# lucidrains/glom-pytorch

Hardware: NVIDIA H100
Metric: column-iterations/sec (BxNxLxiters) at dim=512 L=6 224/14 (higher is better)
Workload: dtype bf16

## Files before the change

### glom_pytorch_b200/csrc/tc_common.cuh

```cuda
#pragma once
#include "engine.h"
#include "ptx.cuh"

#include <stdio.h>

namespace glom {

constexpr int BM = 128;
constexpr int BK = 64;
constexpr uint32_t A_STAGE_BYTES = BM * BK * 2;

constexpr int STG_PITCH = 68;
constexpr uint32_t STG_BYTES = 32 * STG_PITCH * 4;
template <int S, int R>
__device__ __forceinline__ void stage_write_step(const float (&acc)[R], float* stg, int warp_in_wg, int lane) {
  const int r = 16 * (warp_in_wg & 1) + (lane >> 2), c = 2 * (lane & 3);
#pragma unroll
  for (int j = 0; j < 8; ++j) {
#pragma unroll
    for (int h = 0; h < 2; ++h)
      *reinterpret_cast<float2*>(stg + (r + 8 * h) * STG_PITCH + 8 * j + c) =
          make_float2(acc[4 * (8 * S + j) + 2 * h], acc[4 * (8 * S + j) + 2 * h + 1]);
  }
}
template <int R>
__device__ __forceinline__ void stage_write(const float (&acc)[R], float* stg, int s, int warp_in_wg, int lane) {
  static_assert(R % 32 == 0 && R <= 128, "m64 x N fragment, N in {64, 128, 256}");
  if (s == 0) stage_write_step<0>(acc, stg, warp_in_wg, lane);
  if constexpr (R >= 64) { if (s == 1) stage_write_step<1>(acc, stg, warp_in_wg, lane); }
  if constexpr (R >= 128) {
    if (s == 2) stage_write_step<2>(acc, stg, warp_in_wg, lane);
    if (s == 3) stage_write_step<3>(acc, stg, warp_in_wg, lane);
  }
}
__device__ __forceinline__ void stage_read(const float* stg, int x, int lane, uint32_t (&v)[32]) {
  const float4* src = reinterpret_cast<const float4*>(stg + lane * STG_PITCH + 32 * x);
#pragma unroll
  for (int q = 0; q < 8; ++q) {
    const float4 f = src[q];
    v[4 * q] = __float_as_uint(f.x); v[4 * q + 1] = __float_as_uint(f.y);
    v[4 * q + 2] = __float_as_uint(f.z); v[4 * q + 3] = __float_as_uint(f.w);
  }
}

template <int N, int TB>
__device__ __forceinline__ void wgmma_kblock(float (&acc)[N / 2], uint32_t a_smem, uint32_t b_smem) {
  const uint64_t ad = wgmma_desc_sw128(a_smem, 16, 1024);
  const uint64_t bd = TB ? wgmma_desc_sw128(b_smem, 8192, 1024) : wgmma_desc_sw128(b_smem, 16, 1024);
#pragma unroll
  for (int k = 0; k < BK / 16; ++k) wgmma_bf16<N, 0, TB>(acc, ad + 2 * k, bd + (TB ? (2048 >> 4) : 2) * k);
}

__device__ __forceinline__ float row_chunk_sumsq(float a, float b, float c, float d) {
  float q = a * a;
  q = fmaf(b, b, q);
  q = fmaf(c, c, q);
  q = fmaf(d, d, q);
  q += __shfl_xor_sync(0xffffffffu, q, 1);
  q += __shfl_xor_sync(0xffffffffu, q, 2);
  q += __shfl_xor_sync(0xffffffffu, q, 4);
  return q;
}

struct K2Chunk {
  int l, L, d, n, row0;
  int prow0;
  int s_bcast;
  bool remap;
  const float* s32_in; const __nv_bfloat16* c_in; const float* pos;
  float* s32_out; __nv_bfloat16* sb_out; __nv_bfloat16* sp_out;
};
template <bool FULL, bool SETTLE = false>
__device__ __forceinline__ void k2_chunk(const uint32_t (&v)[32], const float4 b4, uint8_t* patch, const K2Chunk& k,
                                         int col, int lane, int rows_left, float (&rowsq)[8], uint32_t live = ~0u,
                                         float* rowdsq = nullptr, bool want_dsq = false) {
#pragma unroll
  for (int c = 0; c < 8; ++c)
    *reinterpret_cast<uint4*>(patch + lane * 128 + ((c ^ (lane & 7)) << 4)) =
        make_uint4(v[4 * c], v[4 * c + 1], v[4 * c + 2], v[4 * c + 3]);
  __syncwarp();
  const int c = lane & 7, rsub = lane >> 3;
  const bool top = (k.l == k.L - 1);
  const bool has_td = (k.l >= 1);
  const int ld = k.L * k.d, ldp = (k.L - 1) * k.d;
  const size_t base = ((size_t)k.row0 * k.L + k.l) * k.d + col + c * 4;
  const size_t pbase = ((size_t)k.row0 * (k.L - 1) + (k.l - 1)) * k.d + col + c * 4;
#pragma unroll
  for (int h = 0; h < 2; ++h) {
    float4 sv[4], pp[4];
    uint2 cw[4];
#pragma unroll
    for (int j = 0; j < 4; ++j) {
      const int r = (h * 4 + j) * 4 + rsub;
      sv[j] = make_float4(0.f, 0.f, 0.f, 0.f); pp[j] = sv[j]; cw[j] = make_uint2(0u, 0u);
      if ((FULL || r < rows_left) && (!SETTLE || ((live >> r) & 1u))) {
        size_t so = base + (unsigned)(r * ld);
        if (!SETTLE && k.remap) {
          int sr = k.prow0 + r;
          if (k.n >= 32) { if (sr >= k.n) sr -= k.n; } else sr %= k.n;
          so = (size_t)k.l * k.d + col + c * 4 + (unsigned)(sr * ld);
        }
        sv[j] = k.s_bcast ? __ldg(reinterpret_cast<const float4*>(k.s32_in + (size_t)k.l * k.d + col + c * 4))
                          : __ldcs(reinterpret_cast<const float4*>(k.s32_in + so));
        cw[j] = __ldcs(reinterpret_cast<const uint2*>(k.c_in + so));
        if (has_td) {
          int pr = k.prow0 + r;
          if (k.n >= 32) { if (pr >= k.n) pr -= k.n; } else pr %= k.n;
          pp[j] = __ldg(reinterpret_cast<const float4*>(k.pos + (size_t)pr * k.d + col + c * 4));
        }
      }
    }
#pragma unroll
    for (int j = 0; j < 4; ++j) {
      const int i = h * 4 + j;
      const int r = i * 4 + rsub;
      const float4 acc = *reinterpret_cast<const float4*>(patch + r * 128 + ((c ^ (r & 7)) << 4));
      float o0 = (sv[j].x + (acc.x + b4.x)) + __uint_as_float(cw[j].x << 16);
      float o1 = (sv[j].y + (acc.y + b4.y)) + __uint_as_float(cw[j].x & 0xFFFF0000u);
      float o2 = (sv[j].z + (acc.z + b4.z)) + __uint_as_float(cw[j].y << 16);
      float o3 = (sv[j].w + (acc.w + b4.w)) + __uint_as_float(cw[j].y & 0xFFFF0000u);
      if (top) { o0 = o0 / 3.0f; o1 = o1 / 3.0f; o2 = o2 / 3.0f; o3 = o3 / 3.0f; }
      else { o0 *= 0.25f; o1 *= 0.25f; o2 *= 0.25f; o3 *= 0.25f; }
      const bool store = (FULL || r < rows_left) && (!SETTLE || ((live >> r) & 1u));
      if constexpr (SETTLE) if (want_dsq) {
        const float e0 = store ? o0 - sv[j].x : 0.f, e1 = store ? o1 - sv[j].y : 0.f;
        const float e2 = store ? o2 - sv[j].z : 0.f, e3 = store ? o3 - sv[j].w : 0.f;
        rowdsq[i] += row_chunk_sumsq(e0, e1, e2, e3);
      }
      if (store) {
        const size_t o = base + (unsigned)(r * ld);
        __stcs(reinterpret_cast<float4*>(k.s32_out + o), make_float4(o0, o1, o2, o3));
        *reinterpret_cast<uint2*>(k.sb_out + o) = make_uint2(pack_bf16x2(o0, o1), pack_bf16x2(o2, o3));
        if (has_td)
          *reinterpret_cast<uint2*>(k.sp_out + pbase + (unsigned)(r * ldp)) =
              make_uint2(pack_bf16x2(o0 + pp[j].x, o1 + pp[j].y), pack_bf16x2(o2 + pp[j].z, o3 + pp[j].w));
      } else {
        o0 = o1 = o2 = o3 = 0.f;
      }
      rowsq[i] += row_chunk_sumsq(o0, o1, o2, o3);
    }
  }
  __syncwarp();
}

static inline int encode_map(Launch& ln, CUtensorMap* m, const void* base, int rank, const uint64_t* dims,
                             const uint64_t* strides_bytes , const uint32_t* box, const char* what) {
  cuuint64_t gd[3]; cuuint64_t gs[2]; cuuint32_t bx[3]; cuuint32_t es[3] = {1, 1, 1};
  for (int i = 0; i < rank; ++i) { gd[i] = dims[i]; bx[i] = box[i]; }
  for (int i = 0; i < rank - 1; ++i) gs[i] = strides_bytes[i];
  const CUresult r = ln.enc(m, CU_TENSOR_MAP_DATA_TYPE_BFLOAT16, (cuuint32_t)rank, const_cast<void*>(base), gd, gs, bx, es,
                         CU_TENSOR_MAP_INTERLEAVE_NONE, CU_TENSOR_MAP_SWIZZLE_128B, CU_TENSOR_MAP_L2_PROMOTION_L2_256B,
                         CU_TENSOR_MAP_FLOAT_OOB_FILL_NONE);
  if (r != CUDA_SUCCESS) return ln.fail(GLOM_B200_ERR_CUDA, "cuTensorMapEncodeTiled(%s) failed with CUresult %d", what, (int)r);
  return 0;
}

static inline int map2d(Launch& ln, CUtensorMap* m, const void* base, uint64_t rows, uint64_t cols, uint32_t box_rows,
                        const char* what) {
  const uint64_t dims[2] = {cols, rows};
  const uint64_t strides[1] = {cols * 2};
  const uint32_t box[2] = {(uint32_t)BK, box_rows};
  return encode_map(ln, m, base, 2, dims, strides, box, what);
}

}
```

### glom_pytorch_b200/csrc/tc_kernels.cu

```cuda
#include "gemm_sched.cuh"
#include "tc_common.cuh"

#include <stdio.h>
#include <stdlib.h>
#include <string.h>

#include <type_traits>

namespace glom {

constexpr int GEMM_CONSUMER_WARPS = 8;
constexpr int GEMM_THREADS = 128 + 32 * GEMM_CONSUMER_WARPS;
constexpr uint32_t GEMM_PRODUCER_REGS = 40;
constexpr uint32_t GEMM_CONSUMER_REGS = 232;

__device__ unsigned long long g_kernel_clk[PROF_KINDS][8];


template <int MODE, int BN>
struct GemmCfg {
  static constexpr int PARTS = (BN == 256) ? 4 : 2;
  static constexpr int PART_COLS = BN / PARTS;
  static constexpr int THREADS = GEMM_THREADS;
  static constexpr uint32_t B_STAGE_BYTES = BN * BK * 2;
  static constexpr uint32_t STAGE_BYTES = A_STAGE_BYTES + B_STAGE_BYTES;
  static_assert(MODE >= 0 && MODE <= 2, "0 = GEMM1+GELU, 1 = GEMM2+combine, 2 = tokeniser");
  static constexpr int STAGES = (BN == 256) ? 3 : (BN == 128) ? 4 : 5;
  static constexpr uint32_t OUT_BOX_BYTES = 64 * BK * 2;
  static constexpr uint32_t PATCH_BYTES = 4096;
  static constexpr size_t EPI_BYTES = (MODE == 0) ? 2 * (BN / 64) * (size_t)OUT_BOX_BYTES
                                                  : 4 * (size_t)STG_BYTES + (size_t)GEMM_CONSUMER_WARPS * PATCH_BYTES + 4 * 32 * 4;
  static constexpr size_t SMEM_BYTES = 1024  + (size_t)STAGES * STAGE_BYTES + EPI_BYTES + 256 ;
  static_assert(SMEM_BYTES <= 232448, "over the 227 KB of shared memory a block may opt in to");
};

__device__ __forceinline__ void tok_chunk(const uint32_t (&v)[32], const float4 b4, uint8_t* patch, float* dst,
                                          size_t pitch, int lane, int rows_left) {
#pragma unroll
  for (int c = 0; c < 8; ++c)
    *reinterpret_cast<uint4*>(patch + lane * 128 + ((c ^ (lane & 7)) << 4)) =
        make_uint4(v[4 * c], v[4 * c + 1], v[4 * c + 2], v[4 * c + 3]);
  __syncwarp();
  const int c = lane & 7, rsub = lane >> 3;
#pragma unroll
  for (int i = 0; i < 8; ++i) {
    const int r = i * 4 + rsub;
    const float4 a = *reinterpret_cast<const float4*>(patch + r * 128 + ((c ^ (r & 7)) << 4));
    if (r < rows_left)
      *reinterpret_cast<float4*>(dst + (size_t)r * pitch + c * 4) = make_float4(a.x + b4.x, a.y + b4.y, a.z + b4.z, a.w + b4.w);
  }
  __syncwarp();
}

template <int MODE>
__device__ __forceinline__ bool settle_skip(const GemmParams& p, const TileInfo& t) {
  if (p.block_frozen[t.m_blk]) return true;
  return MODE == 0 && t.z == 0 && p.block_fresh != nullptr && !p.block_fresh[t.m_blk];
}

template <int MODE, int BN, bool CNT, bool SETTLE = false>
__global__ void __launch_bounds__(GEMM_THREADS, 1)
gemm_kernel(const __grid_constant__ CUtensorMap map_a0,
            const __grid_constant__ CUtensorMap map_a1,
            const __grid_constant__ CUtensorMap map_a2,
            const __grid_constant__ CUtensorMap map_b,
            const __grid_constant__ CUtensorMap map_out,
            const GemmParams p) {
  using Cfg = GemmCfg<MODE, BN>;
  constexpr int STAGES = Cfg::STAGES;
  constexpr bool RED = MODE != 2 && !SETTLE;
  extern __shared__ uint8_t smem_raw[];
  uint8_t* smem = smem_raw + ((1024u - (smem_u32(smem_raw) & 1023u)) & 1023u);
  uint8_t* epi = smem + (size_t)STAGES * Cfg::STAGE_BYTES;
  float* stg_all = reinterpret_cast<float*>(epi);
  uint8_t* patches = epi + 4 * STG_BYTES;
  float* xch = reinterpret_cast<float*>(patches + (size_t)GEMM_CONSUMER_WARPS * Cfg::PATCH_BYTES);
  uint64_t* full_bar = reinterpret_cast<uint64_t*>(epi + Cfg::EPI_BYTES);
  uint64_t* empty_bar = full_bar + STAGES;

  const int warp = threadIdx.x >> 5;
  const int lane = threadIdx.x & 31;
  constexpr int W_TMA = 0;
  constexpr int W_CONSUMER0 = 4;
  const int cta_rank = (int)(blockIdx.x & 1);
  const int cluster_id = blockIdx.x >> 1;
  const int num_clusters = gridDim.x >> 1;

  if (warp == W_TMA && lane == 0) {
    tma_prefetch_desc(&map_a0);
    tma_prefetch_desc(&map_b);
    if (MODE == 0) { tma_prefetch_desc(&map_a1); tma_prefetch_desc(&map_a2); tma_prefetch_desc(&map_out); }
    for (int i = 0; i < STAGES; ++i) { mbar_init(&full_bar[i], 1); mbar_init(&empty_bar[i], 2 * GEMM_CONSUMER_WARPS); }
    fence_barrier_init();
  }
  cluster_sync_all();
  pdl_launch_dependents();
  pdl_wait();
  const bool clk_thread = blockIdx.x == 0 && warp == W_TMA && lane == 0;
  ClockSample* clk_s = reinterpret_cast<ClockSample*>(empty_bar + STAGES);
  if (clk_thread) *clk_s = clock_sample_begin();
  const bool cnt_cta = CNT && blockIdx.x == 0;
  unsigned long long* const cnt = g_kernel_clk[MODE == 0 ? PROF_GEMM1 : MODE == 1 ? PROF_GEMM2 : PROF_TOKENIZE];
  unsigned long long w0 = 0, w1 = 0;
#define GLOM_CNT_WAIT(acc, stmt) do { if (cnt_cta) { const long long t_ = clock64(); stmt; acc += (unsigned long long)(clock64() - t_); } else { stmt; } } while (0)

  if (warp < W_CONSUMER0) {
    setmaxnreg_dec<GEMM_PRODUCER_REGS>();
    if (warp == W_TMA) {
      const uint32_t elected = elect_one();
      int stage = 0; uint32_t phase = 0;
      const uint32_t smem0 = smem_u32(smem);
      const uint64_t pol_first = l2_policy_evict_first();
      const int kbg_n = 4 * p.d / BK;
      const int blk_skip = (p.m128 - 1) * kbg_n;
      for (int it = 0, tile; (tile = sched_tile<MODE>(p, cluster_id, num_clusters, it)) >= 0; ++it) {
        const TileInfo t = decode_tile<MODE, RED>(p, tile);
        if constexpr (SETTLE) { if (settle_skip<MODE>(p, t)) continue; }
        const CUtensorMap* amap;
        int a_col, b_row;
        if (MODE == 0) {
          const int l = t.z >> 1;
          if (t.z == 0) { amap = &map_a0; a_col = 0; }
          else if (t.z & 1) { amap = &map_a2; a_col = l * p.d; }
          else { amap = &map_a1; a_col = (l - 1) * p.d; }
          b_row = t.z * 4 * p.d + t.n_blk * BN;
        } else if (MODE == 1) {
          amap = &map_a0; a_col = 0;
          b_row = t.z * p.d + t.n_blk * BN;
        } else {
          amap = &map_a0; a_col = 0;
          b_row = t.n_blk * BN;
        }
        const int a_row = t.m_blk * 256 + cta_rank * BM;
        const int blk0 = (2 * t.z * p.m128 + (a_row >> 7)) * kbg_n;
        int td_skip = blk_skip;
        if constexpr (RED && MODE == 1) {
          if (p.num_m_rep > 0 && t.z + 1 >= p.remap_l) td_skip -= ((a_row >> 7) - (a_row >> 7) % p.h_period) * kbg_n;
        }
        for (int kb = 0; kb < t.num_kb; ++kb) {
          GLOM_CNT_WAIT(w0, mbar_wait(&empty_bar[stage], phase ^ 1));
          if (elected) {
            const uint32_t sa = smem0 + (uint32_t)stage * Cfg::STAGE_BYTES;
            uint64_t* bar = &full_bar[stage];
            mbar_arrive_expect_tx(bar, Cfg::STAGE_BYTES);
            if (MODE == 1) {
              const int blk = blk0 + kb + (kb >= kbg_n ? td_skip : 0);
              tma_load_2d_hint(sa, amap, bar, 0, blk * BM, pol_first);
            } else {
              tma_load_2d(sa, amap, bar, a_col + kb * BK, a_row);
            }
            const uint32_t b_half = (uint32_t)cta_rank * (BN / 2);
            tma_load_2d_multicast(sa + A_STAGE_BYTES + b_half * BK * 2, &map_b, bar, kb * BK, b_row + (int)b_half, 0x3);
          }
          __syncwarp();
          if (++stage == STAGES) { stage = 0; phase ^= 1; }
        }
      }
      if (cnt_cta && elected) atomicAdd(&cnt[4], w0);
    }
  } else {
    setmaxnreg_inc<GEMM_CONSUMER_REGS>();
    const int cw = warp - W_CONSUMER0;
    const int wg = cw >> 2, wi = cw & 3;
    const int pair = cw >> 1, x = cw & 1;
    float* stg = stg_all + pair * (STG_BYTES / 4);
    uint8_t* patch = patches + (size_t)cw * Cfg::PATCH_BYTES;
    float* xch_p = xch + pair * 32;
    const uint32_t smem0 = smem_u32(smem);
    const uint64_t pol_stream = l2_policy_evict_first();
    const bool st_issuer = (threadIdx.x & 127) == 0;
    const uint32_t out_wg = smem_u32(epi) + (uint32_t)wg * (BN / 64) * Cfg::OUT_BOX_BYTES;
    const uint32_t st_row = (uint32_t)(16 * wi + 8 * ((lane >> 3) & 1) + (lane & 7)) * 128;
    const int st_jx = lane >> 4, st_sw = lane & 7;
    const uint32_t empty_peer = mapa_shared(smem_u32(empty_bar), (uint32_t)cta_rank ^ 1u);
    auto release = [&](int slot) {
      __syncwarp();
      if (lane == 0) { mbar_arrive(&empty_bar[slot]); mbar_arrive_cluster(empty_peer + 8u * (uint32_t)slot); }
    };
    int stage = 0; uint32_t phase = 0;
    float acc[BN / 2];
    for (int it = 0, tile; (tile = sched_tile<MODE>(p, cluster_id, num_clusters, it)) >= 0; ++it) {
      const TileInfo t = decode_tile<MODE, RED>(p, tile);
      if constexpr (SETTLE) { if (settle_skip<MODE>(p, t)) continue; }
      const int row0 = t.m_blk * 256 + cta_rank * BM + pair * 32;
      const int rows_left = p.rows - row0;
      uint32_t live = ~0u;
      if constexpr (SETTLE && MODE == 1)
        live = __ballot_sync(0xffffffffu, row0 + lane < p.rows && !p.frozen[(row0 + lane) / p.n]);
      bool remap = false;
      if constexpr (RED && MODE == 1) remap = p.num_m_rep > 0 && t.z >= p.remap_l;
      if (MODE == 1 && lane < rows_left) {
        const int src_row = remap ? (row0 + lane) % p.n : row0 + lane;
        const size_t o = ((size_t)src_row * p.L + t.z) * p.d + t.n_blk * BN + x * (BN / 2);
#pragma unroll
        for (int c = 0; c < BN / 2; c += 32) {
          if (!p.s_bcast) prefetch_l2(p.s32_in + o + c);
          if ((c & 63) == 0) prefetch_l2(p.c_in + o + c);
        }
      }
#pragma unroll
      for (int i = 0; i < BN / 2; ++i) acc[i] = 0.f;
      int prev = -1;
      for (int kb = 0; kb < t.num_kb; ++kb) {
        GLOM_CNT_WAIT(w0, mbar_wait(&full_bar[stage], phase));
        const uint32_t sa = smem0 + (uint32_t)stage * Cfg::STAGE_BYTES;
        wgmma_fence_regs(acc);
        wgmma_fence();
        wgmma_kblock<BN, 0>(acc, sa + (uint32_t)wg * (A_STAGE_BYTES / 2), sa + A_STAGE_BYTES);
        wgmma_commit();
        wgmma_wait<1>();
        wgmma_fence_regs(acc);
        if (prev >= 0) release(prev);
        prev = stage;
        if (++stage == STAGES) { stage = 0; phase ^= 1; }
      }
      wgmma_wait<0>();
      wgmma_fence_regs(acc);
      release(prev);
      const long long busy_t0 = cnt_cta ? clock64() : 0;
      if constexpr (MODE == 0) {
        const int wrow0 = t.m_blk * 256 + cta_rank * BM + 64 * wg;
        if (wrow0 < p.rows) {
          const int hblk0 = (t.z * p.m128 + (t.m_blk * 2 + cta_rank)) * (4 * p.d / BK) + t.n_blk * (BN / BK);
          const float* bias = p.bias + (size_t)t.z * 4 * p.d + t.n_blk * BN + 2 * (lane & 3);
          uint32_t pk[BN / 4];
#pragma unroll
          for (int s = 0; s < BN / 64; ++s) {
#pragma unroll
            for (int j = 0; j < 8; ++j) {
              const float2 b = __ldg(reinterpret_cast<const float2*>(bias + 64 * s + 8 * j));
#pragma unroll
              for (int h = 0; h < 2; ++h)
                pk[16 * s + 2 * j + h] = gelu_pair_bf16(acc[4 * (8 * s + j) + 2 * h], acc[4 * (8 * s + j) + 2 * h + 1], b.x, b.y);
            }
          }
          if (st_issuer) bulk_wait_group_read<0>();
          named_bar_sync(1 + wg, 128);
#pragma unroll
          for (int s = 0; s < BN / 64; ++s)
#pragma unroll
            for (int q = 0; q < 4; ++q)
              stmatrix_x4(out_wg + (uint32_t)s * Cfg::OUT_BOX_BYTES + st_row + ((uint32_t)((2 * q + st_jx) ^ st_sw) << 4),
                          pk[16 * s + 4 * q], pk[16 * s + 4 * q + 1], pk[16 * s + 4 * q + 2], pk[16 * s + 4 * q + 3]);
          fence_proxy_async_smem();
          named_bar_sync(1 + wg, 128);
          if (st_issuer) {
#pragma unroll
            for (int s = 0; s < BN / 64; ++s)
              tma_store_2d_hint(&map_out, out_wg + (uint32_t)s * Cfg::OUT_BOX_BYTES, 0, (hblk0 + s) * BM + 64 * wg, pol_stream);
            bulk_commit_group();
          }
        }
      } else {
#pragma unroll 1
        for (int s = 0; s < BN / 64; ++s) {
          stage_write(acc, stg, s, wi, lane);
          named_bar_sync(1 + pair, 64);
          uint32_t v[32];
          stage_read(stg, x, lane, v);
          const int cc = 64 * s + 32 * x;
          if (MODE == 2) {
            float* trow = p.tok_out + (size_t)row0 * p.d + t.n_blk * BN + cc;
            const float4 b4 = __ldg(reinterpret_cast<const float4*>(p.bias + t.n_blk * BN + cc + (lane & 7) * 4));
            tok_chunk(v, b4, patch, trow, (size_t)p.d, lane, rows_left);
          } else {
            K2Chunk kc;
            kc.l = t.z; kc.L = p.L; kc.d = p.d; kc.n = p.n; kc.row0 = row0; kc.prow0 = row0 % p.n; kc.s_bcast = p.s_bcast;
            kc.remap = remap;
            kc.s32_in = p.s32_in; kc.c_in = p.c_in; kc.pos = p.pos;
            kc.s32_out = p.s32_out; kc.sb_out = p.sb_out; kc.sp_out = p.sp_out;
            const int col = t.n_blk * BN + cc;
            const float4 b4 = __ldg(reinterpret_cast<const float4*>(p.bias + (size_t)t.z * p.d + col + (lane & 7) * 4));
            float rowsq[8], rowdsq[8];
#pragma unroll
            for (int i = 0; i < 8; ++i) rowsq[i] = rowdsq[i] = 0.f;
            const bool want_dsq = SETTLE && p.dsq_out != nullptr;
            if (rows_left >= 32) k2_chunk<true, SETTLE>(v, b4, patch, kc, col, lane, 32, rowsq, live, rowdsq, want_dsq);
            else k2_chunk<false, SETTLE>(v, b4, patch, kc, col, lane, rows_left, rowsq, live, rowdsq, want_dsq);
            int part = cc / Cfg::PART_COLS;
            bool writer = true;
            if (Cfg::PART_COLS == 64) {
              float* dxch = reinterpret_cast<float*>(patches + (size_t)(cw | 1) * Cfg::PATCH_BYTES);
              if (x == 1 && (lane & 7) == 0) {
#pragma unroll
                for (int i = 0; i < 8; ++i) xch_p[i * 4 + (lane >> 3)] = rowsq[i];
                if (want_dsq) {
#pragma unroll
                  for (int i = 0; i < 8; ++i) dxch[i * 4 + (lane >> 3)] = rowdsq[i];
                }
              }
              named_bar_sync(1 + pair, 64);
              if (x == 0) {
#pragma unroll
                for (int i = 0; i < 8; ++i) rowsq[i] += xch_p[i * 4 + (lane >> 3)];
                if (want_dsq) {
#pragma unroll
                  for (int i = 0; i < 8; ++i) rowdsq[i] += dxch[i * 4 + (lane >> 3)];
                }
              }
              writer = x == 0;
            }
            if (writer && (lane & 7) == 0) {
              const size_t po = ((size_t)row0 * p.L + t.z) * p.nparts + t.n_blk * Cfg::PARTS + part;
              float* nsq = p.nsq_out + po;
              const int ldn = p.L * p.nparts;
#pragma unroll
              for (int i = 0; i < 8; ++i) {
                const int r = i * 4 + (lane >> 3);
                if (r < rows_left && (!SETTLE || ((live >> r) & 1u))) {
                  nsq[(unsigned)(r * ldn)] = rowsq[i];
                  if (want_dsq) p.dsq_out[po + (unsigned)(r * ldn)] = rowdsq[i];
                }
              }
            }
          }
          named_bar_sync(1 + pair, 64);
        }
      }
      if (cnt_cta) w1 += (unsigned long long)(clock64() - busy_t0);
    }
    if (cnt_cta && cw == 0 && lane == 0) { atomicAdd(&cnt[2], w0); atomicAdd(&cnt[6], w1); }
    if (MODE == 0 && st_issuer) bulk_wait_group<0>();
  }
#undef GLOM_CNT_WAIT

  cluster_sync_all();
  if (clk_thread) clock_sample_end(*clk_s, g_kernel_clk[MODE == 0 ? PROF_GEMM1 : MODE == 1 ? PROF_GEMM2 : PROF_TOKENIZE]);
}

constexpr int ATTN_CONSUMER_WARPS = 8;
constexpr int ATTN_THREADS = 128 + 32 * ATTN_CONSUMER_WARPS;
constexpr uint32_t ATTN_PRODUCER_REGS = 56;
constexpr uint32_t ATTN_CONSUMER_REGS = 224;
constexpr int ATTN_SCALE_WARPS = 3;
constexpr float ATTN_BOUND_MAX = 96.f;
constexpr int ATTN_SINGLE_PASS_MAX = 576;
constexpr int ATTN_PASS_KEYS = 512;

template <int KEYS>
struct AttnCfg {
  static_assert(KEYS == 128 || KEYS == 256, "S block = one wgmma N");
  static constexpr int MAX_KB = (KEYS == 256) ? 1 : 5;
  static constexpr uint32_t SLOT_BYTES = A_STAGE_BYTES + (uint32_t)KEYS * BK * 2;
  static_assert(SLOT_BYTES >= 4 * 8192, "a slot holds a V chunk");
};

struct AttnParams {
  int n, L, d;
  int attend_self, mask_side, mask_d2_max;
  int n_pad16, n_pad64, nkb, nchunk;
  int num_stages;
  int ntiles, num_items;
  int nparts;
  const float* nsq;
  __nv_bfloat16* c_out;
  float scale;
  int key0, nk, pass_first, pass_last;
  float* o_acc;
  float* ml_acc;
  const int* frozen;
  int l_full;
};

constexpr size_t attn_fixed_smem(int nchunk, int n_pad16) {
  return 1024  + (size_t)nchunk * A_STAGE_BYTES + (size_t)n_pad16 * (2 * 2 * 4 + 4) + 256;
}
static_assert(attn_fixed_smem(4, 256) + 3 * AttnCfg<256>::SLOT_BYTES <= 232448, "n = 256: three 48 KB slots");
static_assert(attn_fixed_smem(9, 576) + 2 * AttnCfg<128>::SLOT_BYTES <= 232448, "n = 576: two 32 KB slots");

__device__ __forceinline__ float attn_row_norm(const float* ns, int nparts) {
  float ss = 0.f;
  if ((nparts & 3) == 0 && nparts <= 16) {
    float4 q[4];
#pragma unroll
    for (int i = 0; i < 4; ++i)
      q[i] = 4 * i < nparts ? __ldg(reinterpret_cast<const float4*>(ns) + i) : make_float4(0.f, 0.f, 0.f, 0.f);
#pragma unroll
    for (int i = 0; i < 4; ++i) ss = (((ss + q[i].x) + q[i].y) + q[i].z) + q[i].w;
  } else {
    for (int i = 0; i < nparts; ++i) ss += ns[i];
  }
  return sqrtf(ss);
}

template <int KEYS, bool CNT, bool SETTLE = false>
__global__ void __launch_bounds__(ATTN_THREADS, 1)
attn_kernel(const __grid_constant__ CUtensorMap map_q,
            const __grid_constant__ CUtensorMap map_k,
            const __grid_constant__ CUtensorMap map_v,
            const AttnParams p) {
  using Cfg = AttnCfg<KEYS>;
  constexpr uint32_t SLOT = Cfg::SLOT_BYTES;
  extern __shared__ uint8_t smem_raw[];
  uint8_t* smem = smem_raw + ((1024u - (smem_u32(smem_raw) & 1023u)) & 1023u);
  uint8_t* p_smem = smem;
  uint8_t* stages = p_smem + (size_t)p.nchunk * A_STAGE_BYTES;
  float* sc = reinterpret_cast<float*>(stages + (size_t)p.num_stages * SLOT);
  uint32_t* key_hw = reinterpret_cast<uint32_t*>(sc + 4 * p.n_pad16);
  uint64_t* full_bar = reinterpret_cast<uint64_t*>(key_hw + p.n_pad16);
  uint64_t* empty_bar = full_bar + p.num_stages;
  uint64_t* sc_full = empty_bar + p.num_stages;
  uint64_t* sc_empty = sc_full + 2;
  ClockSample* clk_s = reinterpret_cast<ClockSample*>(sc_empty + 2);

  const int warp = threadIdx.x >> 5;
  const int lane = threadIdx.x & 31;
  constexpr int W_TMA = 0;
  constexpr int W_CONSUMER0 = 4;
  const int nsub = (p.d + 255) / 256;
  const int per_img = p.ntiles * (SETTLE ? p.L : p.l_full);
  const int full_items = p.num_items - p.ntiles * (p.L - p.l_full);
  auto item_bl = [&](int it, int& b, int& l) {
    if (SETTLE) { b = it / per_img; l = (it % per_img) / p.ntiles; }
    else attn_item(it, full_items, per_img, p.ntiles, p.l_full, b, l);
  };
  const int nkb = (KEYS == 256) ? 1 : p.nkb;
  constexpr float LOG2E = 1.4426950408889634f;

  if (warp == W_TMA && lane == 0) {
    tma_prefetch_desc(&map_q); tma_prefetch_desc(&map_k); tma_prefetch_desc(&map_v);
    for (int i = 0; i < p.num_stages; ++i) { mbar_init(&full_bar[i], 1); mbar_init(&empty_bar[i], ATTN_CONSUMER_WARPS); }
    for (int i = 0; i < 2; ++i) { mbar_init(&sc_full[i], ATTN_SCALE_WARPS); mbar_init(&sc_empty[i], ATTN_CONSUMER_WARPS); }
    fence_barrier_init();
  }
  __syncthreads();
  pdl_launch_dependents();
  pdl_wait();
  const bool clk_thread = blockIdx.x == 0 && warp == W_TMA && lane == 0;
  if (clk_thread) *clk_s = clock_sample_begin();
  const bool cnt_cta = CNT && blockIdx.x == 0;
  unsigned long long* const cnt = g_kernel_clk[PROF_ATTN];
  unsigned long long w0 = 0, w1 = 0, w2 = 0;
#define GLOM_CNT_WAIT(acc, stmt) do { if (cnt_cta) { const long long t_ = clock64(); stmt; acc += (unsigned long long)(clock64() - t_); } else { stmt; } } while (0)

  if (warp < W_CONSUMER0) {
    setmaxnreg_dec<ATTN_PRODUCER_REGS>();
    if (warp == W_TMA) {
      const uint32_t elected = elect_one();
      int stage = 0; uint32_t phase = 0;
      const uint32_t stages0 = smem_u32(stages);
      for (int it = blockIdx.x; it < p.num_items; it += gridDim.x) {
        int b, l;
        item_bl(it, b, l);
        if constexpr (SETTLE) { if (p.frozen[b]) continue; }
        const int q0 = (it % p.ntiles) * BM;
        for (int kb = 0; kb < nkb; ++kb) {
          for (int dc = 0; dc < p.d / BK; ++dc) {
// ... 230 lines not shown
              uint32_t* ptr = p_word(rbase + 8 * h, kb * KEYS + col);
              const uint32_t wv = *ptr;
              *ptr = pack_bf16x2(__uint_as_float(wv << 16) * f, __uint_as_float(wv & 0xFFFF0000u) * f);
            }
          }
        }
      }
      float l_pass[2];
#pragma unroll
      for (int h = 0; h < 2; ++h) {
        l_pass[h] = l_run[h] + __shfl_xor_sync(0xffffffffu, l_run[h], 1);
        l_pass[h] += __shfl_xor_sync(0xffffffffu, l_pass[h], 2);
      }
      fence_proxy_async_smem();
      named_bar_sync(2 + wg, 128);
      const long long cnt_t1 = cnt_cta ? clock64() : 0;
      const unsigned long long cnt_w1 = w0;
      if (cnt_cta) w1 += (unsigned long long)(cnt_t1 - cnt_t0) - (cnt_w1 - cnt_w0);

      size_t acc_row[2];
      float inv_l[2], f_old[2] = {0.f, 0.f}, f_new[2] = {1.f, 1.f};
#pragma unroll
      for (int h = 0; h < 2; ++h) {
        acc_row[h] = (img_row0 + (size_t)qi[h]) * p.L + l;
        inv_l[h] = 1.0f / l_pass[h];
        if (multi) {
          float m_acc = NEG_INF, l_acc = 0.f;
          if (!p.pass_first && qi[h] < p.n) {
            const float2 ml = *reinterpret_cast<const float2*>(p.ml_acc + acc_row[h] * 2);
            m_acc = ml.x; l_acc = ml.y;
          }
          float m_pass = exact_max ? m_run[h] : row_bound[h];
          if (l_pass[h] == 0.f) m_pass = NEG_INF;
          const float m_new = fmaxf(m_acc, m_pass);
          f_old[h] = (m_acc == NEG_INF) ? 0.f : ex2_approx(m_acc - m_new);
          f_new[h] = (m_pass == NEG_INF) ? 0.f : ex2_approx(m_pass - m_new);
          const float l_new = l_acc * f_old[h] + l_pass[h] * f_new[h];
          inv_l[h] = p.pass_last ? 1.0f / l_new : 1.0f;
          __syncwarp();
          if (!p.pass_last && (lane & 3) == 0 && qi[h] < p.n)
            *reinterpret_cast<float2*>(p.ml_acc + acc_row[h] * 2) = make_float2(m_new, l_new);
        }
      }

#pragma unroll 1
      for (int sp = 0; sp < nsub; ++sp) {
        float o[128];
#pragma unroll
        for (int i = 0; i < 128; ++i) o[i] = 0.f;
        int prev = -1;
        for (int kc = 0; kc < p.nchunk; ++kc) {
          GLOM_CNT_WAIT(w0, mbar_wait(&full_bar[stage], phase));
          const uint32_t sa = stages0 + (uint32_t)stage * SLOT;
          wgmma_fence_regs(o);
          wgmma_fence();
          wgmma_kblock<256, 1>(o, p0 + (uint32_t)kc * A_STAGE_BYTES + (uint32_t)wg * (A_STAGE_BYTES / 2), sa);
          wgmma_commit();
          wgmma_wait<1>();
          wgmma_fence_regs(o);
          if (prev >= 0) { __syncwarp(); if (lane == 0) mbar_arrive(&empty_bar[prev]); }
          prev = stage;
          if (++stage == p.num_stages) { stage = 0; phase ^= 1; }
        }
        wgmma_wait<0>();
        wgmma_fence_regs(o);
        __syncwarp();
        if (lane == 0) mbar_arrive(&empty_bar[prev]);
        if (multi) {
#pragma unroll
          for (int i = 0; i < 128; i += 2) {
            const int h = (i >> 1) & 1;
            const int col = sp * 256 + 8 * (i >> 2) + cq;
            if (col >= p.d || qi[h] >= p.n) continue;
            float v0 = o[i], v1 = o[i + 1];
            float2* accp = reinterpret_cast<float2*>(p.o_acc + acc_row[h] * p.d + col);
            float2 prev = make_float2(0.f, 0.f);
            if (!p.pass_first) prev = *accp;
            v0 = v0 * f_new[h] + prev.x * f_old[h];
            v1 = v1 * f_new[h] + prev.y * f_old[h];
            if (!p.pass_last) { *accp = make_float2(v0, v1); continue; }
            *reinterpret_cast<uint32_t*>(p.c_out + acc_row[h] * p.d + col) = pack_bf16x2(v0 * inv_l[h], v1 * inv_l[h]);
          }
        } else {
          const int q = lane & 3;
          const bool b1 = q & 1, b2 = q & 2;
#pragma unroll
          for (int h = 0; h < 2; ++h) {
            __nv_bfloat16* crow = p.c_out + acc_row[h] * p.d + sp * 256 + 8 * q;
            const bool row_ok = qi[h] < p.n;
#pragma unroll
            for (int g = 0; g < 8; ++g) {
              uint32_t a[4];
#pragma unroll
              for (int t = 0; t < 4; ++t)
                a[t] = pack_bf16x2(o[4 * (4 * g + t) + 2 * h] * inv_l[h], o[4 * (4 * g + t) + 2 * h + 1] * inv_l[h]);
#pragma unroll
              for (int pr = 0; pr < 2; ++pr) {
                const uint32_t r = __shfl_xor_sync(0xffffffffu, b1 ? a[2 * pr] : a[2 * pr + 1], 1);
                if (b1) a[2 * pr] = r; else a[2 * pr + 1] = r;
              }
#pragma unroll
              for (int pr = 0; pr < 2; ++pr) {
                const uint32_t r = __shfl_xor_sync(0xffffffffu, b2 ? a[pr] : a[2 + pr], 2);
                if (b2) a[pr] = r; else a[2 + pr] = r;
              }
              if (row_ok && sp * 256 + 32 * g < p.d)
                *reinterpret_cast<uint4*>(crow + 32 * g) = make_uint4(a[0], a[1], a[2], a[3]);
            }
          }
        }
      }
      if (cnt_cta) w2 += (unsigned long long)(clock64() - cnt_t1) - (w0 - cnt_w1);
      ++k;
    }
    if (cnt_cta && cw == 0 && lane == 0) { atomicAdd(&cnt[5], w0); atomicAdd(&cnt[6], w1); atomicAdd(&cnt[7], w2); }
  }
#undef GLOM_CNT_WAIT

  __syncthreads();
  if (clk_thread) clock_sample_end(*clk_s, g_kernel_clk[PROF_ATTN]);
}

cudaError_t tc_kernel_clocks(unsigned long long* out , bool reset) {
  cudaError_t e = cudaMemcpyFromSymbol(out, g_kernel_clk, sizeof(unsigned long long) * PROF_KINDS * 8);
  if (e == cudaSuccess && reset) {
    static const unsigned long long zeros[PROF_KINDS * 8] = {};
    e = cudaMemcpyToSymbol(g_kernel_clk, zeros, sizeof(zeros));
  }
  return e;
}

template <int MODE, int BN, bool CNT, bool SETTLE = false>
static cudaError_t launch_gemm_impl(const CUtensorMap& a0, const CUtensorMap& a1, const CUtensorMap& a2, const CUtensorMap& bm,
                                    const CUtensorMap& out, const GemmParams& p, int num_sms, cudaStream_t st);

static bool count_waits() {
  static const bool on = [] { const char* ev = getenv("GLOM_B200_WAIT_COUNTERS"); return ev && ev[0] == '1'; }();
  return on;
}

template <int MODE, int BN>
static cudaError_t launch_gemm(const CUtensorMap& a0, const CUtensorMap& a1, const CUtensorMap& a2, const CUtensorMap& bm,
                               const CUtensorMap& out, const GemmParams& p, int num_sms, cudaStream_t st) {
  if constexpr (MODE != 2) {
    if (p.block_frozen) return launch_gemm_impl<MODE, BN, false, true>(a0, a1, a2, bm, out, p, num_sms, st);
  }
  if (count_waits()) return launch_gemm_impl<MODE, BN, true>(a0, a1, a2, bm, out, p, num_sms, st);
  return launch_gemm_impl<MODE, BN, false>(a0, a1, a2, bm, out, p, num_sms, st);
}

template <int MODE, int BN, bool CNT, bool SETTLE>
static cudaError_t launch_gemm_impl(const CUtensorMap& a0, const CUtensorMap& a1, const CUtensorMap& a2, const CUtensorMap& bm,
                                    const CUtensorMap& out, const GemmParams& p, int num_sms, cudaStream_t st) {
  using Cfg = GemmCfg<MODE, BN>;
  static SmemOptIn optin;
  if (cudaError_t e = optin.ensure(gemm_kernel<MODE, BN, CNT, SETTLE>, Cfg::SMEM_BYTES)) return e;
  cudaLaunchConfig_t cfg{};
  cfg.blockDim = dim3(Cfg::THREADS);
  cfg.dynamicSmemBytes = Cfg::SMEM_BYTES;
  cfg.stream = st;
  cudaLaunchAttribute attr[2];
  attr[0].id = cudaLaunchAttributeProgrammaticStreamSerialization;
  attr[0].val.programmaticStreamSerializationAllowed = 1;
  attr[1].id = cudaLaunchAttributeClusterDimension;
  attr[1].val.clusterDim.x = 2; attr[1].val.clusterDim.y = 1; attr[1].val.clusterDim.z = 1;
  static std::atomic<int> co_resident[64];
  int dev = 0;
  if (cudaError_t e = cudaGetDevice(&dev)) return e;
  if (dev < 0 || dev >= 64) return cudaErrorInvalidDevice;
  int occ = co_resident[dev].load(std::memory_order_relaxed);
  if (occ == 0) {
    int dev_sms = 0;
    if (cudaError_t e = cudaDeviceGetAttribute(&dev_sms, cudaDevAttrMultiProcessorCount, dev)) return e;
    cfg.gridDim = dim3(2 * (dev_sms / 2));
    cfg.attrs = &attr[1]; cfg.numAttrs = 1;
    if (cudaError_t e = cudaOccupancyMaxActiveClusters(&occ, gemm_kernel<MODE, BN, CNT, SETTLE>, &cfg)) return e;
    if (occ < 1) return cudaErrorInvalidConfiguration;
    co_resident[dev].store(occ, std::memory_order_relaxed);
  }
  const int max_pairs = occ < num_sms / 2 ? occ : num_sms / 2;
  cfg.attrs = attr; cfg.numAttrs = 2;
  const int pairs = p.num_tiles < max_pairs ? p.num_tiles : max_pairs;
  cfg.gridDim = dim3(2 * pairs);
  return cudaLaunchKernelEx(&cfg, gemm_kernel<MODE, BN, CNT, SETTLE>, a0, a1, a2, bm, out, p);
}

template <int KEYS, bool CNT, bool SETTLE = false>
static cudaError_t launch_attn_impl(const CUtensorMap& mq, const CUtensorMap& mk, const CUtensorMap& mv, const AttnParams& ap,
                                    size_t smem, int ctas, cudaStream_t st) {
  static SmemOptIn optin;
  if (cudaError_t e = optin.ensure(attn_kernel<KEYS, CNT, SETTLE>, smem)) return e;
  cudaLaunchConfig_t acfg{};
  acfg.gridDim = dim3(ctas); acfg.blockDim = dim3(ATTN_THREADS); acfg.dynamicSmemBytes = smem; acfg.stream = st;
  cudaLaunchAttribute aattr[1];
  aattr[0].id = cudaLaunchAttributeProgrammaticStreamSerialization;
  aattr[0].val.programmaticStreamSerializationAllowed = 1;
  acfg.attrs = aattr; acfg.numAttrs = 1;
  return cudaLaunchKernelEx(&acfg, attn_kernel<KEYS, CNT, SETTLE>, mq, mk, mv, ap);
}

static int launch_attention(const Geometry& g, const Bf16Buffers& b, int l_full, Launch& ln) {
  const int d = g.d, L = g.L, n = g.n;
  const int npass = (n <= ATTN_SINGLE_PASS_MAX) ? 1 : (n + ATTN_PASS_KEYS - 1) / ATTN_PASS_KEYS;
  if (npass > 1 && !b.attn_acc)
    return ln.fail(GLOM_B200_ERR_CUDA, "consensus for n = %d columns needs the key-pass scratch buffer (workspace too old?)", n);
  const int keys = (npass == 1 && (n + 15) / 16 * 16 > 128 && (n + 15) / 16 * 16 <= 256) ? 256 : 128;
  CUtensorMap mq, mk, mv;
  const uint64_t dims[3] = {(uint64_t)L * d, (uint64_t)n, (uint64_t)g.B};
  const uint64_t strides[2] = {(uint64_t)L * d * 2, (uint64_t)n * L * d * 2};
  const uint32_t boxq[3] = {(uint32_t)BK, (uint32_t)BM, 1}, boxk[3] = {(uint32_t)BK, (uint32_t)keys, 1};
  const uint32_t boxv[3] = {(uint32_t)BK, 64, 1};
  GLOM_TRY(encode_map(ln, &mq, b.sb_in, 3, dims, strides, boxq, "attn.q"));
  GLOM_TRY(encode_map(ln, &mk, b.sb_in, 3, dims, strides, boxk, "attn.k"));
  GLOM_TRY(encode_map(ln, &mv, b.sb_in, 3, dims, strides, boxv, "attn.v"));
  const bool cnt = count_waits();
  cudaStream_t st = ln.st;
  for (int pass = 0; pass < npass; ++pass) {
    AttnParams ap{};
    ap.n = n; ap.L = L; ap.d = d;
    ap.attend_self = g.attend_self; ap.mask_side = g.mask_side; ap.mask_d2_max = g.mask_d2_max;
    ap.key0 = npass == 1 ? 0 : pass * ATTN_PASS_KEYS;
    ap.nk = npass == 1 ? n : (n - ap.key0 < ATTN_PASS_KEYS ? n - ap.key0 : ATTN_PASS_KEYS);
    ap.pass_first = pass == 0; ap.pass_last = pass == npass - 1;
    ap.o_acc = b.attn_acc;
    ap.ml_acc = b.attn_acc ? b.attn_acc + (size_t)g.rows * L * d : nullptr;
    ap.n_pad16 = (ap.nk + 15) / 16 * 16;
    ap.n_pad64 = (ap.nk + 63) / 64 * 64;
    ap.nkb = (ap.n_pad16 + keys - 1) / keys;
    ap.nchunk = ap.n_pad64 / 64;
    ap.nparts = g.nparts;
    ap.nsq = b.nsq_in;
    ap.c_out = b.c;
    ap.scale = 1.0f / sqrtf((float)d);
    ap.ntiles = (n + BM - 1) / BM;
    ap.l_full = l_full;
    ap.num_items = ap.ntiles * (l_full * g.B + L - l_full);
    ap.frozen = b.frozen;
    const uint32_t slot = keys == 256 ? AttnCfg<256>::SLOT_BYTES : AttnCfg<128>::SLOT_BYTES;
    const size_t fixed = attn_fixed_smem(ap.nchunk, ap.n_pad16);
    const size_t max_smem = 232448;
    int stages = 4;
    while (stages > 0 && fixed + (size_t)stages * slot > max_smem) --stages;
    if (stages < 2 || ap.nkb > (keys == 256 ? AttnCfg<256>::MAX_KB : AttnCfg<128>::MAX_KB))
      return ln.fail(GLOM_B200_ERR_CUDA, "consensus pass of %d keys does not fit shared memory", ap.nk);
    ap.num_stages = stages;
    const size_t smem = fixed + (size_t)stages * slot;
    const int ctas = ap.num_items < ln.num_sms ? ap.num_items : ln.num_sms;
    ProfScope scope(ln.prof, PROF_ATTN, st);
    cudaError_t e;
    if (b.frozen) e = keys == 256 ? launch_attn_impl<256, false, true>(mq, mk, mv, ap, smem, ctas, st)
                                  : launch_attn_impl<128, false, true>(mq, mk, mv, ap, smem, ctas, st);
    else if (keys == 256) e = cnt ? launch_attn_impl<256, true>(mq, mk, mv, ap, smem, ctas, st)
                                          : launch_attn_impl<256, false>(mq, mk, mv, ap, smem, ctas, st);
    else e = cnt ? launch_attn_impl<128, true>(mq, mk, mv, ap, smem, ctas, st)
                         : launch_attn_impl<128, false>(mq, mk, mv, ap, smem, ctas, st);
    GLOM_TRY(ln.launched(e, "attn_kernel launch"));
  }
  return 0;
}

int step_bf16(const Geometry& g, const Bf16Buffers& b, int step_index, Launch& ln) {
  const int d = g.d, L = g.L, n = g.n, rows = g.rows, num_sms = ln.num_sms;
  cudaStream_t st = ln.st;
  CUtensorMap mh, mh_out;
  const int m128 = (rows + BM - 1) / BM;
  const uint64_t h_rows = (uint64_t)g.G * m128 * (4 * d / BK) * BM;
  GLOM_TRY(map2d(ln, &mh, b.h, h_rows, BK, BM, "H"));
  GLOM_TRY(map2d(ln, &mh_out, b.h, h_rows, BK, 64, "H out"));
  CUtensorMap mx, msb, msp, mw1, mw2;
  GLOM_TRY(map2d(ln, &mx, b.xb, rows, d, BM, "Xb"));
  GLOM_TRY(map2d(ln, &msb, b.sb_in, rows, (uint64_t)L * d, BM, "Sb"));
  GLOM_TRY(map2d(ln, &msp, b.sp_in, rows, (uint64_t)(L - 1) * d, BM, "Sp"));
  GLOM_TRY(map2d(ln, &mw1, b.w1, (uint64_t)g.G * 4 * d, d, 128, "W1p"));
  GLOM_TRY(map2d(ln, &mw2, b.w2, (uint64_t)L * d, (uint64_t)8 * d, (uint32_t)g.bn2 / 2, "W2p"));
  {
    GemmParams p{};
    p.rows = rows; p.d = d; p.L = L; p.n = n; p.G = g.G;
    p.z0 = (step_index > 0 && g.G > 1 && !b.block_fresh) ? 1 : 0;
    p.num_m = (rows + 255) / 256; p.num_n = 4 * d / 256; p.num_tiles = (g.G - p.z0) * p.num_m * p.num_n;
    p.bias = b.b1; p.m128 = m128;
    p.frozen = b.frozen; p.block_frozen = b.block_frozen; p.block_fresh = b.block_fresh;
    if (b.ii_reduce) set_reduced(p, g.G, rep_row_blocks(n), [&](int z) { return ii_k1_full(z, step_index); });
    ProfScope scope(ln.prof, PROF_GEMM1, st);
    GLOM_TRY(ln.launched(launch_gemm<0, 256>(mx, msb, msp, mw1, mh_out, p, num_sms, st), "gemm1 launch"));
  }
  GLOM_TRY(launch_attention(g, b, b.ii_reduce ? ii_k3_full_levels(step_index) : L, ln));
  {
    GemmParams p{};
    p.rows = rows; p.d = d; p.L = L; p.n = n; p.G = g.G;
    p.num_m = (rows + 255) / 256; p.num_n = d / g.bn2; p.z0 = 0; p.num_tiles = L * p.num_m * p.num_n;
    p.n_half = p.num_m * p.num_n;
    p.m128 = m128;
    p.bias = b.b2; p.s32_in = b.s32_in; p.s_bcast = b.s32_in_bcast; p.c_in = b.c; p.pos = b.pos;
    p.s32_out = b.s32_out; p.sb_out = b.sb_out; p.sp_out = b.sp_out; p.nsq_out = b.nsq_out; p.nparts = g.nparts;
    p.frozen = b.frozen; p.block_frozen = b.block_frozen; p.dsq_out = b.dsq_out;
    if (b.ii_reduce) {
      set_reduced(p, L, rep_row_blocks(n), [&](int l) { return ii_k2_full(l, step_index); });
      p.n_half = (L - 1 <= step_index ? p.num_m : p.num_m_rep) * p.num_n;
      p.remap_l = step_index; p.h_period = rep_h_blocks(n);
    }
    cudaError_t e;
    ProfScope scope(ln.prof, PROF_GEMM2, st);
    if (g.bn2 == 256) e = launch_gemm<1, 256>(mh, mh, mh, mw2, mh, p, num_sms, st);
    else if (g.bn2 == 128) e = launch_gemm<1, 128>(mh, mh, mh, mw2, mh, p, num_sms, st);
    else e = launch_gemm<1, 64>(mh, mh, mh, mw2, mh, p, num_sms, st);
    GLOM_TRY(ln.launched(e, "gemm2 launch"));
  }
// ... 25 lines not shown
```

Before: 67.98 million.

## Read GEMM2 epilogue straight from staging buffer and add a pipeline stage

```diff
diff --git a/glom_pytorch_b200/csrc/tc_common.cuh b/glom_pytorch_b200/csrc/tc_common.cuh
--- a/glom_pytorch_b200/csrc/tc_common.cuh
+++ b/glom_pytorch_b200/csrc/tc_common.cuh
@@ -143,6 +143,66 @@
   __syncwarp();
 }
 
+template <bool FULL>
+__device__ __forceinline__ void k2_chunk_direct(const float* stg, const float4 b4, const K2Chunk& k, int col, int lane,
+                                                int rows_left, float (&rowsq)[8]) {
+  const int c = lane & 7, rsub = lane >> 3;
+  const bool top = (k.l == k.L - 1);
+  const bool has_td = (k.l >= 1);
+  const int ld = k.L * k.d, ldp = (k.L - 1) * k.d;
+  const size_t base = ((size_t)k.row0 * k.L + k.l) * k.d + col + c * 4;
+  const size_t pbase = ((size_t)k.row0 * (k.L - 1) + (k.l - 1)) * k.d + col + c * 4;
+#pragma unroll
+  for (int h = 0; h < 2; ++h) {
+    float4 sv[4], pp[4];
+    uint2 cw[4];
+#pragma unroll
+    for (int j = 0; j < 4; ++j) {
+      const int r = (h * 4 + j) * 4 + rsub;
+      sv[j] = make_float4(0.f, 0.f, 0.f, 0.f); pp[j] = sv[j]; cw[j] = make_uint2(0u, 0u);
+      if (FULL || r < rows_left) {
+        size_t so = base + (unsigned)(r * ld);
+        if (k.remap) {
+          int sr = k.prow0 + r;
+          if (k.n >= 32) { if (sr >= k.n) sr -= k.n; } else sr %= k.n;
+          so = (size_t)k.l * k.d + col + c * 4 + (unsigned)(sr * ld);
+        }
+        sv[j] = k.s_bcast ? __ldg(reinterpret_cast<const float4*>(k.s32_in + (size_t)k.l * k.d + col + c * 4))
+                          : __ldcs(reinterpret_cast<const float4*>(k.s32_in + so));
+        cw[j] = __ldcs(reinterpret_cast<const uint2*>(k.c_in + so));
+        if (has_td) {
+          int pr = k.prow0 + r;
+          if (k.n >= 32) { if (pr >= k.n) pr -= k.n; } else pr %= k.n;
+          pp[j] = __ldg(reinterpret_cast<const float4*>(k.pos + (size_t)pr * k.d + col + c * 4));
+        }
+      }
+    }
+#pragma unroll
+    for (int j = 0; j < 4; ++j) {
+      const int i = h * 4 + j;
+      const int r = i * 4 + rsub;
+      const float4 acc = *reinterpret_cast<const float4*>(stg + r * STG_PITCH + c * 4);
+      float o0 = (sv[j].x + (acc.x + b4.x)) + __uint_as_float(cw[j].x << 16);
+      float o1 = (sv[j].y + (acc.y + b4.y)) + __uint_as_float(cw[j].x & 0xFFFF0000u);
+      float o2 = (sv[j].z + (acc.z + b4.z)) + __uint_as_float(cw[j].y << 16);
+      float o3 = (sv[j].w + (acc.w + b4.w)) + __uint_as_float(cw[j].y & 0xFFFF0000u);
+      if (top) { o0 = o0 / 3.0f; o1 = o1 / 3.0f; o2 = o2 / 3.0f; o3 = o3 / 3.0f; }
+      else { o0 *= 0.25f; o1 *= 0.25f; o2 *= 0.25f; o3 *= 0.25f; }
+      if (FULL || r < rows_left) {
+        const size_t o = base + (unsigned)(r * ld);
+        __stcs(reinterpret_cast<float4*>(k.s32_out + o), make_float4(o0, o1, o2, o3));
+        *reinterpret_cast<uint2*>(k.sb_out + o) = make_uint2(pack_bf16x2(o0, o1), pack_bf16x2(o2, o3));
+        if (has_td)
+          *reinterpret_cast<uint2*>(k.sp_out + pbase + (unsigned)(r * ldp)) =
+              make_uint2(pack_bf16x2(o0 + pp[j].x, o1 + pp[j].y), pack_bf16x2(o2 + pp[j].z, o3 + pp[j].w));
+      } else {
+        o0 = o1 = o2 = o3 = 0.f;
+      }
+      rowsq[i] += row_chunk_sumsq(o0, o1, o2, o3);
+    }
+  }
+}
+
 static inline int encode_map(Launch& ln, CUtensorMap* m, const void* base, int rank, const uint64_t* dims,
                              const uint64_t* strides_bytes , const uint32_t* box, const char* what) {
   cuuint64_t gd[3]; cuuint64_t gs[2]; cuuint32_t bx[3]; cuuint32_t es[3] = {1, 1, 1};
diff --git a/glom_pytorch_b200/csrc/tc_kernels.cu b/glom_pytorch_b200/csrc/tc_kernels.cu
--- a/glom_pytorch_b200/csrc/tc_kernels.cu
+++ b/glom_pytorch_b200/csrc/tc_kernels.cu
@@ -17,7 +17,7 @@
 __device__ unsigned long long g_kernel_clk[PROF_KINDS][8];
 
 
-template <int MODE, int BN>
+template <int MODE, int BN, bool SETTLE = false>
 struct GemmCfg {
   static constexpr int PARTS = (BN == 256) ? 4 : 2;
   static constexpr int PART_COLS = BN / PARTS;
@@ -25,13 +25,18 @@
   static constexpr uint32_t B_STAGE_BYTES = BN * BK * 2;
   static constexpr uint32_t STAGE_BYTES = A_STAGE_BYTES + B_STAGE_BYTES;
   static_assert(MODE >= 0 && MODE <= 2, "0 = GEMM1+GELU, 1 = GEMM2+combine, 2 = tokeniser");
-  static constexpr int STAGES = (BN == 256) ? 3 : (BN == 128) ? 4 : 5;
+  static constexpr bool DIRECT = MODE == 1 && BN == 256 && !SETTLE;
+  static constexpr int STAGES = DIRECT ? 4 : (BN == 256) ? 3 : (BN == 128) ? 4 : 5;
   static constexpr uint32_t OUT_BOX_BYTES = 64 * BK * 2;
   static constexpr uint32_t PATCH_BYTES = 4096;
   static constexpr size_t EPI_BYTES = (MODE == 0) ? 2 * (BN / 64) * (size_t)OUT_BOX_BYTES
-                                                  : 4 * (size_t)STG_BYTES + (size_t)GEMM_CONSUMER_WARPS * PATCH_BYTES + 4 * 32 * 4;
-  static constexpr size_t SMEM_BYTES = 1024  + (size_t)STAGES * STAGE_BYTES + EPI_BYTES + 256 ;
+                                    : DIRECT ? 4 * (size_t)STG_BYTES
+                                             : 4 * (size_t)STG_BYTES + (size_t)GEMM_CONSUMER_WARPS * PATCH_BYTES + 4 * 32 * 4;
+  static constexpr size_t BAR_BYTES = 128;
+  static constexpr size_t SMEM_BYTES = DIRECT ? 1024 + (size_t)STAGES * STAGE_BYTES + EPI_BYTES
+                                              : 1024  + (size_t)STAGES * STAGE_BYTES + EPI_BYTES + 256 ;
   static_assert(SMEM_BYTES <= 232448, "over the 227 KB of shared memory a block may opt in to");
+  static_assert(!DIRECT || 2 * STAGES * 8 + sizeof(ClockSample) <= BAR_BYTES, "barriers + clock sample in BAR_BYTES");
 };
 
 __device__ __forceinline__ void tok_chunk(const uint32_t (&v)[32], const float4 b4, uint8_t* patch, float* dst,
@@ -66,7 +71,7 @@
             const __grid_constant__ CUtensorMap map_b,
             const __grid_constant__ CUtensorMap map_out,
             const GemmParams p) {
-  using Cfg = GemmCfg<MODE, BN>;
+  using Cfg = GemmCfg<MODE, BN, SETTLE>;
   constexpr int STAGES = Cfg::STAGES;
   constexpr bool RED = MODE != 2 && !SETTLE;
   extern __shared__ uint8_t smem_raw[];
@@ -76,6 +81,9 @@
   uint8_t* patches = epi + 4 * STG_BYTES;
   float* xch = reinterpret_cast<float*>(patches + (size_t)GEMM_CONSUMER_WARPS * Cfg::PATCH_BYTES);
   uint64_t* full_bar = reinterpret_cast<uint64_t*>(epi + Cfg::EPI_BYTES);
+  if constexpr (Cfg::DIRECT) {
+    if (smem - smem_raw >= (ptrdiff_t)Cfg::BAR_BYTES) full_bar = reinterpret_cast<uint64_t*>(smem_raw);
+  }
   uint64_t* empty_bar = full_bar + STAGES;
 
   const int warp = threadIdx.x >> 5;
@@ -165,7 +173,8 @@
     const int pair = cw >> 1, x = cw & 1;
     float* stg = stg_all + pair * (STG_BYTES / 4);
     uint8_t* patch = patches + (size_t)cw * Cfg::PATCH_BYTES;
-    float* xch_p = xch + pair * 32;
+    float* xch_p = Cfg::DIRECT ? stg + 64 : xch + pair * 32;
+    constexpr int XCH_STRIDE = Cfg::DIRECT ? STG_PITCH : 1;
     const uint32_t smem0 = smem_u32(smem);
     const uint64_t pol_stream = l2_policy_evict_first();
     const bool st_issuer = (threadIdx.x & 127) == 0;
@@ -257,7 +266,7 @@
           stage_write(acc, stg, s, wi, lane);
           named_bar_sync(1 + pair, 64);
           uint32_t v[32];
-          stage_read(stg, x, lane, v);
+          if constexpr (!Cfg::DIRECT) stage_read(stg, x, lane, v);
           const int cc = 64 * s + 32 * x;
           if (MODE == 2) {
             float* trow = p.tok_out + (size_t)row0 * p.d + t.n_blk * BN + cc;
@@ -275,15 +284,20 @@
 #pragma unroll
             for (int i = 0; i < 8; ++i) rowsq[i] = rowdsq[i] = 0.f;
             const bool want_dsq = SETTLE && p.dsq_out != nullptr;
-            if (rows_left >= 32) k2_chunk<true, SETTLE>(v, b4, patch, kc, col, lane, 32, rowsq, live, rowdsq, want_dsq);
-            else k2_chunk<false, SETTLE>(v, b4, patch, kc, col, lane, rows_left, rowsq, live, rowdsq, want_dsq);
+            if constexpr (Cfg::DIRECT) {
+              if (rows_left >= 32) k2_chunk_direct<true>(stg + 32 * x, b4, kc, col, lane, 32, rowsq);
+              else k2_chunk_direct<false>(stg + 32 * x, b4, kc, col, lane, rows_left, rowsq);
+            } else {
+              if (rows_left >= 32) k2_chunk<true, SETTLE>(v, b4, patch, kc, col, lane, 32, rowsq, live, rowdsq, want_dsq);
+              else k2_chunk<false, SETTLE>(v, b4, patch, kc, col, lane, rows_left, rowsq, live, rowdsq, want_dsq);
+            }
             int part = cc / Cfg::PART_COLS;
             bool writer = true;
             if (Cfg::PART_COLS == 64) {
               float* dxch = reinterpret_cast<float*>(patches + (size_t)(cw | 1) * Cfg::PATCH_BYTES);
               if (x == 1 && (lane & 7) == 0) {
 #pragma unroll
-                for (int i = 0; i < 8; ++i) xch_p[i * 4 + (lane >> 3)] = rowsq[i];
+                for (int i = 0; i < 8; ++i) xch_p[(i * 4 + (lane >> 3)) * XCH_STRIDE] = rowsq[i];
                 if (want_dsq) {
 #pragma unroll
                   for (int i = 0; i < 8; ++i) dxch[i * 4 + (lane >> 3)] = rowdsq[i];
@@ -292,7 +306,7 @@
               named_bar_sync(1 + pair, 64);
               if (x == 0) {
 #pragma unroll
-                for (int i = 0; i < 8; ++i) rowsq[i] += xch_p[i * 4 + (lane >> 3)];
+                for (int i = 0; i < 8; ++i) rowsq[i] += xch_p[(i * 4 + (lane >> 3)) * XCH_STRIDE];
                 if (want_dsq) {
 #pragma unroll
                   for (int i = 0; i < 8; ++i) rowdsq[i] += dxch[i * 4 + (lane >> 3)];
@@ -829,7 +843,7 @@
 template <int MODE, int BN, bool CNT, bool SETTLE>
 static cudaError_t launch_gemm_impl(const CUtensorMap& a0, const CUtensorMap& a1, const CUtensorMap& a2, const CUtensorMap& bm,
                                     const CUtensorMap& out, const GemmParams& p, int num_sms, cudaStream_t st) {
-  using Cfg = GemmCfg<MODE, BN>;
+  using Cfg = GemmCfg<MODE, BN, SETTLE>;
   static SmemOptIn optin;
   if (cudaError_t e = optin.ensure(gemm_kernel<MODE, BN, CNT, SETTLE>, Cfg::SMEM_BYTES)) return e;
   cudaLaunchConfig_t cfg{};
```

New measurement: 69.03 million (median of 6 runs). 1.5% higher.
